# domainxz/top-k-rec

Hardware: AMD Instinct MI355X
Metric: BPR training triplets/sec (sampler + plan + step), MovieLens-10M shape (higher is better)
Workload: dtype f32

## Files before the change

### include/tkr.h

```cpp
#ifndef TKR_H
#define TKR_H
#include <stdint.h>

#ifdef __cplusplus
extern "C" {
#endif

#define TKR_VERSION 120
#define TKR_OK 0
#define TKR_E_INVAL (-1)
#define TKR_E_UNSUPPORTED (-2)
#define TKR_E_IO (-3)
#define TKR_E_PARSE (-4)
#define TKR_E_NOMEM (-5)

int tkr_version(void);
int tkr_lab_build(void);

int tkr_plan_team(int32_t batch_size);
int tkr_plan_max_blocks(int32_t batch_size);
int tkr_sample_plan(const int32_t* tr_users, int32_t n_tr, const int32_t* row_ptr, const int32_t* pos_cols,
                    const int32_t* cols_sorted, int32_t n_users, int32_t n_items, uint64_t seed,
                    uint64_t first_triplet, const int64_t* ctl, int32_t n_batches, int32_t batch_size,
                    int32_t* ucnt, int32_t* icnt, uint32_t* touch_u, uint32_t* touch_i, int32_t* out_u,
// ... 13 lines not shown
    float* b;
    float* msb;
    int32_t n_users, n_items, k;
    int32_t mode;
    float lu, li, lj, lb;
    float lr;
    float rho, eps;
    int32_t opt;
} tkr_bpr_state;

int tkr_bpr_run(const tkr_bpr_state* st, int32_t* rec, const int32_t* occ, const int32_t* hdr,
                int32_t batch_size, int32_t n_batches, float* loss_out, void* stream);

typedef struct {
    void* U;
    void* msU;
    void* tailU;
    uint32_t* rdU;
    void* V;
    void* msV;
    void* tailV;
    uint32_t* rdV;
    int32_t n_users, n_items, k;
    int32_t mode;
    float lu, li, lj, lb;
    float lr, rho, eps;
    int32_t opt;
    int32_t item_bufs;
} tkr_flow_state;
int32_t tkr_flow_row_granules(int32_t k);
int32_t tkr_flow_ctl_words(void);
#define TKR_FLOW_CTL_STATUS 1026
#define TKR_FLOW_CTL_SPINS 1027
int tkr_bpr_flow_run(const tkr_flow_state* st, const int32_t* prec, const int32_t* pocc, int32_t batch_size,
                     int32_t n_batches, uint32_t* ctl, float* loss_out, int32_t waves_per_cu, void* stream);

int32_t tkr_bpr_own_owners(int32_t n_items, int32_t k);
int32_t tkr_bpr_own_owners_shared(int32_t n_items, int32_t k, int32_t share);
int tkr_sample_plan_owned(const int32_t* tr_users, int32_t n_tr, const int32_t* row_ptr, const int32_t* pos_cols,
                          const int32_t* cols_sorted, int32_t n_users, int32_t n_items, uint64_t seed, uint64_t first_triplet,
                          int32_t n_batches, int32_t batch_size, int32_t* ucnt, int32_t* icnt, uint32_t* touch_u,
                          uint32_t* touch_i, int32_t* out_u, int32_t* out_i, int32_t* out_j, int32_t* task, int32_t* occ,
                          int32_t* occt, int32_t* prec, int32_t* pocc, int32_t n_owner, int32_t* ohdr, int32_t ohdr_stride,
                          void* stream);
int tkr_bpr_own_run(const tkr_flow_state* st, const int32_t* prec, const int32_t* pocc, const int32_t* occt, const int32_t* ohdr,
                    int32_t ohdr_stride, int32_t n_owner, int32_t batch_size, int32_t first_batch, int32_t n_batches, uint32_t* ctl, float* loss_out,
                    int32_t owner_waves, void* xch, uint32_t epoch, void* stream);
typedef struct tkr_plan_call {
    const int32_t *tr_users, *row_ptr, *pos_cols, *cols_sorted;
    int32_t *ucnt, *icnt;
    uint32_t *touch_u, *touch_i;
    int32_t *out_u, *out_i, *out_j, *task, *occ, *occt, *prec, *pocc, *ohdr;
    uint64_t seed, first_triplet;
    int32_t n_tr, n_users, n_items, n_batches, batch_size, n_owner, ohdr_stride, reserved;
} tkr_plan_call;
int tkr_bpr_own_plan_run(const tkr_plan_call* plan, const tkr_flow_state* st, int32_t first_batch, int32_t n_batches, uint32_t* ctl,
                         float* loss_out, int32_t owner_waves, void* xch, uint32_t epoch, void* ev_before, void* ev_after, void* stream);
int tkr_bpr_own_run_between(void* ev_before, void* ev_after, const tkr_flow_state* st, const int32_t* prec, const int32_t* pocc,
                            const int32_t* occt, const int32_t* ohdr, int32_t ohdr_stride, int32_t n_owner, int32_t batch_size,
                            int32_t first_batch, int32_t n_batches, uint32_t* ctl, float* loss_out, int32_t owner_waves, void* xch,
                            uint32_t epoch, void* stream);

typedef struct {
    float* U;
    float* msU;
    float* I;
// ... 246 lines not shown
```

### top-k-rec_amd/csrc/bpr_own.hip

```cpp
#include "flow_task.h"
#ifndef TKR_TAG_NAP
#define TKR_TAG_NAP 4
#endif
#ifdef TKR_PLAN_STAMP
namespace tkr { __device__ unsigned long long own_k1_prof[32]; }
#define K1_STAMP(i) do { if (blockIdx.x == 0 && threadIdx.x == 0) tkr::own_k1_prof[i] = __builtin_amdgcn_s_memrealtime(); } while (0)
#define K1_STAMP_ITEMS(i) do { if (blockIdx.x == 0 && threadIdx.x == 256) tkr::own_k1_prof[i] = __builtin_amdgcn_s_memrealtime(); } while (0)
#endif
#include "plan_parts.h"

namespace tkr {

struct PlanArgs {
    const int32_t *tr_users, *row_ptr, *pos_cols, *cols_sorted;
    int32_t *ucnt, *icnt;
    uint32_t *touch_u, *touch_i;
    int32_t *out_u, *out_i, *out_j;
    int4* task;
    int2* occ;
    int32_t* occt;
    int4 *prec, *pocc;
    int32_t* ohdr;
    uint64_t seed, first_triplet;
    uint32_t n_tr, n_items;
// ... 11 lines not shown
        }
        lds_poke(flag, ok);
    }
    __syncthreads();
    const bool ok = lds_peek(flag) != 0u;
    __syncthreads();
    return ok;
}

constexpr uint32_t kOwnInvalid = 0xffffffffu;

__host__ __device__ inline size_t plan_scratch_bytes(int B, int npad_items, int n_owner, int own_words) {
    size_t a = (size_t)npad_items * 8 + (kWideThreads / TKR_WAVE + 1) * 4;
    if (a < (size_t)(256 + 512) * 8 + 64) a = (size_t)(256 + 512) * 8 + 64;
    const size_t pb = (size_t)3 * B * 20 + (size_t)4 * n_owner * (own_words + 1) + (kWideThreads / TKR_WAVE + 1) * 4 + 16 + (size_t)3 * B * 32;
    return ((a > pb ? a : pb) + 15) & ~(size_t)15;
}

template <bool PLAN>
__device__ __forceinline__ int4 plan_ld(const int4* __restrict__ prec, const __amdgpu_buffer_rsrc_t& prec_r, size_t idx16) {
    if constexpr (PLAN) {
        const v4u x = __builtin_amdgcn_raw_buffer_load_b128(prec_r, (int)(idx16 * 16), 0, kAuxLoad);
        return make_int4((int)x.x, (int)x.y, (int)x.z, (int)x.w);
    } else {
        return prec[idx16];
    }
}
constexpr int kDotWin = 1024;

struct OwnQueue {
    uint32_t head;
    uint32_t total;
    uint32_t arrival;
    uint32_t head_batch;
};

struct QueueMap {
    const uint32_t* pre;
    const uint32_t* start;
    uint32_t slots_per_batch;
    __device__ __forceinline__ uint32_t locate(uint32_t pos, uint32_t& cur, int lane) const {
        uint32_t before;
        for (;;) {
            const uint32_t v = pre[cur + 1 + lane];
            const unsigned long long m = __ballot(v > pos);
            if (m) {
                const int f = __ffsll((long long)m) - 1;
                before = f ? (uint32_t)bcast_i((int)v, f - 1) : pre[cur];
                cur += f;
                break;
            }
            cur += TKR_WAVE;
        }
        return cur * slots_per_batch + start[cur] + (pos - before);
    }
};

template <bool PLAN>
struct UserTicketSrc {
    uint32_t ticket;
    int home, queues;
    uint32_t total;
    uint32_t B;
    const int4* __restrict__ prec;
    __amdgpu_buffer_rsrc_t prec_r;
    __device__ __forceinline__ void prefetch(NextTask& nx, int lane) {
        const u64 i64 = (u64)(uint32_t)bcast_i((int)ticket, 0) * (uint32_t)queues + (uint32_t)home;
// ... 3 lines not shown
        if (idx == 0xffffffffu) { nx.idx = idx; return; }
        nx.idx = idx + 2u * B * (idx / B);
        if (lane < 8) nx.w = plan_ld<PLAN>(prec, prec_r, (size_t)nx.idx * 8 + lane);
    }
};

template <int NP>
__device__ __forceinline__ void lds_row_read(const float* row, int lane, bool sgd, float (&own)[2 * NP], float (&ms)[2 * NP], Own& o) {
    constexpr int KP = NP * 128;
#pragma unroll
    for (int q = 0; q < NP; ++q) {
        const float2 a = *reinterpret_cast<const float2*>(row + q * 128 + 2 * lane);
        own[2 * q] = a.x; own[2 * q + 1] = a.y;
        if (!sgd) {
            const float2 m = *reinterpret_cast<const float2*>(row + KP + q * 128 + 2 * lane);
            ms[2 * q] = m.x; ms[2 * q + 1] = m.y;
        }
    }
    const float4 t = *reinterpret_cast<const float4*>(row + 2 * KP);
    const float2 t2 = *reinterpret_cast<const float2*>(row + 2 * KP + 4);
    o.b = t.x; o.msb = t.y;
    o.exp[0] = __float_as_uint(t.z); o.exp[1] = __float_as_uint(t.w);
    o.exp[2] = __float_as_uint(t2.x); o.exp[3] = __float_as_uint(t2.y);
}

struct ItemRow {
    const u64 *own_p, *own_ms, *own_tail;
    const uint32_t* own_rd;
    uint32_t ver;
    bool from_lds;
    const volatile uint32_t* tag;
    const float* row;
    int halves;
    bool rd_staged;
    uint32_t rd_val;
};

template <int NP>
__device__ __forceinline__ bool item_own_wait(const FlowTables& T, int lane, const ItemRow& r, bool sgd, float (&own)[2 * NP], float (&ms)[2 * NP],
                                              Own& o, uint32_t* ctl, uint32_t& spins) {
    if (r.from_lds) {
        uint32_t waited = 0;
        while (lds_peek(r.tag) != r.ver) {
#if TKR_TAG_NAP > 0
            __builtin_amdgcn_s_sleep(TKR_TAG_NAP);
#endif
            if (spin_fail(waited, ctl, 0)) {
                if (waited >= kSpinLimit && lane == 0 && atomicCAS(ctl + kCtlDebug, 0u, 4u) == 0u) {
                    ctl[kCtlDebug + 1] = lds_peek(r.tag); ctl[kCtlDebug + 3] = r.ver;
                }
                return false;
            }
        }
        spins += waited;
        asm volatile("" ::: "memory");
        lds_row_read<NP>(r.row, lane, sgd, own, ms, o);
        o.ok = true;
        if (r.rd_staged) {
            o.rd = r.rd_val;
            return true;
        }
    }
    return flow_own<NP>(T, lane, r.own_p, r.own_ms, r.own_tail, r.own_rd, r.ver, own, ms, o, sgd, ctl, spins, r.halves);
}

template <int NP>
struct LdsOwnStep {
    const FlowTables& T;
    int lane;
    const ItemRow& r;
    bool sgd;
    uint32_t* ctl;
    uint32_t& spins;
    __device__ __forceinline__ bool operator()(float (&own)[2 * NP], float (&ms)[2 * NP], Own& o) {
#ifdef TKR_OWN_PROF
        o.t_own0 = __builtin_amdgcn_s_memtime();
        const bool ok = item_own_wait<NP>(T, lane, r, sgd, own, ms, o, ctl, spins);
        o.t_own1 = __builtin_amdgcn_s_memtime();
        return ok;
#else
        return item_own_wait<NP>(T, lane, r, sgd, own, ms, o, ctl, spins);
#endif
    }
};
struct NoFeed {
    __device__ __forceinline__ void prefetch(NextTask& nx, int) { nx.have = true; }
};

template <int NP>
__device__ __forceinline__ void own_update(const tkr_flow_state& st, bool sgd, const float (&own)[2 * NP], const float (&ms)[2 * NP],
                                           const Own& o, const float (&g)[2 * NP], float gb, float (&pn)[2 * NP], float (&mn)[2 * NP],
                                           float& bn, float& mbn) {
    constexpr int NE = 2 * NP;
    if (sgd) {
// ... 4 lines not shown
    } else {
#pragma unroll
        for (int e = 0; e < NE; ++e) {
            mn[e] = st.rho * ms[e] + (1.f - st.rho) * g[e] * g[e];
            pn[e] = own[e] - st.lr * g[e] * __builtin_amdgcn_rsqf(mn[e] + st.eps);
        }
        mbn = st.rho * o.msb + (1.f - st.rho) * gb * gb;
        bn = o.b - st.lr * gb * __builtin_amdgcn_rsqf(mbn + st.eps);
    }
}

template <int NP>
__device__ __forceinline__ bool own_publish(int lane, bool is_item, uint32_t bmask, bool sgd, u64* tabP, u64* tabM, u64* tabT, size_t woff,
                                            size_t n_rows, int row, int rowk, uint32_t ver, int n_occ, Own& o, const uint32_t* own_rd,
                                            const float (&pn)[2 * NP], const float (&mn)[2 * NP], float bn, float mbn, uint32_t* ctl,
                                            uint32_t& spins, uint32_t readers_per_occ) {
    const uint32_t nv = ver + 1u;
    const uint32_t expect = pick_exp(o, (ver + 1u) & bmask);
    uint32_t waited = 0;
    while ((int32_t)(o.rd - expect) < 0) {
        if (spin_fail(waited, ctl)) {
            if (waited >= kSpinLimit && lane == 0 && atomicCAS(ctl + kCtlDebug, 0u, 2u) == 0u) {
                ctl[kCtlDebug + 1] = o.rd; ctl[kCtlDebug + 2] = expect; ctl[kCtlDebug + 3] = ver; ctl[kCtlDebug + 4] = (uint32_t)rowk;
            }
            return false;
        }
        o.rd = ld_u32(own_rd);
    }
    spins += waited;
#ifdef TKR_OWN_PROF
    o.t_ack = __builtin_amdgcn_s_memtime();
#endif
    store_row<NP>(tabP + woff, lane, pn, nv);
    if (!sgd) store_row<NP>(tabM + woff, lane, mn, nv);
    store_tail(tabT, n_rows, row, bmask, lane, is_item, bn, mbn, o, ver, n_occ, readers_per_occ);
    return true;
}

constexpr int own_threads(int np) { return np == 1 ? 768 : 512; }

template <int NP, bool PLAN = false>
__global__ __launch_bounds__(own_threads(NP), own_threads(NP) / 256) void bpr_own_kernel(
    tkr_flow_state st, const int4* __restrict__ prec , const int4* __restrict__ pocc,
    const int32_t* __restrict__ occt, const int32_t* __restrict__ ohdr , int ohdr_stride,
    int first_batch, int nb, int B, int n_owner, int owner_waves, uint32_t tune, uint32_t* __restrict__ ctl, float* __restrict__ loss_out,
    u64* __restrict__ xch , uint32_t epoch, PlanArgs pa) {
    constexpr int TPB = own_threads(NP);
    constexpr int NE = 2 * NP;
    constexpr int KP = NP * 128;
    constexpr int ROWF = 2 * KP + 8;
    const int lane = threadIdx.x & (TKR_WAVE - 1), wave = threadIdx.x / TKR_WAVE;
    FlowTables T;
    T.tune = 0u;
    T.kp = KP;
    T.ustride = (size_t)st.n_users * T.kp;
    T.istride = (size_t)st.n_items * T.kp;
    T.imask = st.item_bufs == 4 ? 3u : 1u;
    const int item_halves = tail_halves(T.imask);
    T.U = reinterpret_cast<u64*>(st.U); T.msU = reinterpret_cast<u64*>(st.msU); T.tailU = reinterpret_cast<u64*>(st.tailU);
    T.V = reinterpret_cast<u64*>(st.V); T.msV = reinterpret_cast<u64*>(st.msV); T.tailV = reinterpret_cast<u64*>(st.tailV);
    T.rdU = st.rdU; T.rdV = st.rdV;
    const bool sgd = st.opt == 1;
    const bool want_loss = loss_out != nullptr;

    extern __shared__ __attribute__((aligned(16))) unsigned char smem[];
    OwnQueue* q = reinterpret_cast<OwnQueue*>(smem);
    uint32_t* pre = reinterpret_cast<uint32_t*>(smem + sizeof(OwnQueue));
    uint32_t* start = pre + nb + 1 + TKR_WAVE;
    const int rows_here = (st.n_items + n_owner - 1) / n_owner;
    uint32_t* tags = start + nb;
    uint32_t* dotmark = tags + rows_here;
    float* rows = reinterpret_cast<float*>(smem + ((sizeof(OwnQueue) + (size_t)4 * (2 * nb + 1 + TKR_WAVE + rows_here + kDotWin) + 15) & ~(size_t)15));

    const uint32_t me = blockIdx.x;
    bool alive = true;
    int commit_key = -1, commit_total = 0;
#ifdef TKR_PLAN_STAMP
#define PLAN_STAMP(i) do { if ((me == 0 || me == gridDim.x - 1) && threadIdx.x == 0) reinterpret_cast<u64*>(ctl + kCtlProf)[(me ? 16 : 0) + (i)] = __builtin_amdgcn_s_memrealtime(); } while (0)
#else
#define PLAN_STAMP(i) do { } while (0)
#endif
    PLAN_STAMP(0);
    for (int b = threadIdx.x; b < TKR_WAVE; b += TPB) pre[nb + 1 + b] = 0xffffffffu;
    for (int s = threadIdx.x; s < rows_here; s += TPB) tags[s] = kOwnInvalid;
    for (int s = threadIdx.x; s < kDotWin; s += TPB) dotmark[s] = 0u;
    if constexpr (PLAN) {
        static_assert(TPB == kWideThreads, "phase B of the planner is one thread per task slot");
        unsigned char* scratch = reinterpret_cast<unsigned char*>(rows);
        volatile uint32_t* flag = &q->arrival;
        const uint32_t n_plan = (uint32_t)pa.n_plan;
        int4 ct = make_int4(-1, 0, 0, 0);
        int cprev = 0, ctotal = 0;
        if (me < n_plan) {
            const int b = (int)me, n3 = 3 * B;
            int4* task_b = pa.task + (size_t)b * n3;
            int2* occ_b = pa.occ + (size_t)b * n3;
            int32_t* occt_b = pa.occt + (size_t)b * n3;
            const bool split = pa.reg_sort_ok != 0 && pa.npad_items == 512 && B > 128;
            const PlanMirror mir = plan_mirror(scratch + plan_scratch_bytes(B, pa.npad_items, n_owner, pa.own_words), B);
            if (split)
                plan_phase_a_split<TPB>(scratch, b, pa.tr_users, pa.n_tr, pa.row_ptr, pa.pos_cols, pa.cols_sorted, pa.n_items, pa.seed,
                                        pa.first_triplet + (uint64_t)b * (uint64_t)B, B, pa.out_u + (size_t)b * B, pa.out_i + (size_t)b * B,
                                        pa.out_j + (size_t)b * B, task_b, occ_b, occt_b, pa.touch_u, pa.touch_i, mir);
            else
                plan_phase_a<TPB, 256>(scratch, b, pa.tr_users, pa.n_tr, pa.row_ptr, pa.pos_cols, pa.cols_sorted, pa.n_items, pa.seed,
                                       pa.first_triplet + (uint64_t)b * (uint64_t)B, B, pa.npad_items, pa.out_u + (size_t)b * B, pa.out_i + (size_t)b * B,
                                       pa.out_j + (size_t)b * B, task_b, occ_b, occt_b, pa.touch_u, pa.touch_i, pa.reg_sort_ok != 0);
            PLAN_STAMP(1);
            asm volatile("s_waitcnt vmcnt(0)" ::: "memory");
            __syncthreads();
            PLAN_STAMP(2);
            alive = plan_rendezvous<4>(ctl + kCtlPlanA, n_plan, true, ctl, flag);
            PLAN_STAMP(3);
            if (alive) {
                if (split)
                    plan_phase_b_wide<true, true>(scratch, b, B, task_b, occ_b, occt_b, pa.ucnt, pa.icnt, pa.touch_u, pa.touch_i, pa.pocc + (size_t)b * n3,
                                                  pa.prec + (size_t)b * n3 * 8, n_owner, pa.ohdr, ohdr_stride, pa.own_words, ct, cprev, ctotal, mir);
                else
// ... 10 lines not shown
        commit_key = (alive && me < n_plan && (int)threadIdx.x < 3 * B && ct.x != -1 && cprev == -1) ? ct.x : -1;
        commit_total = ctotal;
        PLAN_STAMP(9);
    }
    const bool ticket_wave = wave > owner_waves;
    const int tw = wave - owner_waves - 1, n_tw = TPB / TKR_WAVE - owner_waves - 1;
    const int queues = min(kQueues, max(n_tw, 1) * (int)gridDim.x);
    const int home = ticket_wave ? (int)((me * (uint32_t)n_tw + (uint32_t)tw) % (uint32_t)queues) : 0;
    uint32_t ticket = 0;
    if (ticket_wave) ticket = grab_issue(ctl, lane, home);
    for (int b = threadIdx.x; b < nb; b += TPB) {
        uint32_t h = 0u;
        if (me < (uint32_t)n_owner) {
            if constexpr (PLAN) h = (uint32_t)__hip_atomic_load(ohdr + (size_t)me * ohdr_stride + b, __ATOMIC_RELAXED, __HIP_MEMORY_SCOPE_AGENT);
            else h = (uint32_t)ohdr[(size_t)me * ohdr_stride + b];
        }
        start[b] = h & 0xffffu;
        pre[b + 1] = h >> 16;
    }
    __syncthreads();
    if (wave == 0) {
        const int per = (nb + TKR_WAVE - 1) / TKR_WAVE;
        const int b0 = min(lane * per, nb), b1 = min(b0 + per, nb);
        uint32_t mine = 0;
        for (int b = b0; b < b1; ++b) mine += pre[b + 1];
        uint32_t incl = mine;
#pragma unroll
        for (int d = 1; d < TKR_WAVE; d <<= 1) {
            const uint32_t up = (uint32_t)__shfl_up((int)incl, d);
            if (lane >= d) incl += up;
        }
        uint32_t run = incl - mine;
        for (int b = b0; b < b1; ++b) { run += pre[b + 1]; pre[b + 1] = run; }
        if (lane == TKR_WAVE - 1) { q->total = incl; q->head = 0u; q->head_batch = 0u; }
        if (lane == 0) pre[0] = 0u;
    }
    __syncthreads();

    PLAN_STAMP(10);
    uint32_t spins = 0;
#ifdef TKR_OWN_PROF
    u64 prof[16] = {0, 0, 0, 0, 0, 0, 0, 0, 0, 0, 0, 0, 0, 0, 0, 0};
    u64 tprev = __builtin_amdgcn_s_memtime();
#endif
    const QueueMap qm{pre, start, 3u * (uint32_t)B};
    const __amdgpu_buffer_rsrc_t prec_r = row_rsrc(prec, PLAN ? nb * 3 * B * 128 : 16);
    const uint32_t q_total = q->total;

    auto item_row = [&](const int4 w, ItemRow& r, int& row, int& slot) {
        const int rowk = bcast_i(w.x, 0);
        const uint32_t ver = (uint32_t)bcast_i(w.y, 0);
        const int prev = bcast_i(w.y, 1);
        row = rowk & 0x7fffffff;
        slot = row / n_owner;
        const size_t roff = (size_t)(ver & T.imask) * T.istride + (size_t)row * T.kp;
        r.own_p = T.V + roff; r.own_ms = T.msV + roff;
        r.own_tail = T.tailV + ((size_t)(ver & T.imask) * st.n_items + row) * (2 * item_halves);
        r.own_rd = T.rdV + (T.imask + 1u) * (size_t)row + ((ver + 1u) & T.imask);
        r.ver = ver;
        r.from_lds = prev >= first_batch;
        r.tag = tags + slot;
        r.row = rows + (size_t)slot * ROWF;
        r.halves = item_halves;
        r.rd_staged = false;
        r.rd_val = 0u;
    };

    constexpr uint32_t kItemReaders = 2u;
    if (wave <= owner_waves) {
        uint32_t cur = 0;
        while (alive) {
            uint32_t pos = 0;
            if (lane == 0) pos = atomicAdd(&q->head, 1u);
            pos = (uint32_t)bcast_i((int)pos, 0);
            if (pos >= q_total) break;
            const uint32_t idx = qm.locate(pos, cur, lane);
            if (lane == 0) atomicMax(&q->head_batch, cur);
            int4 w = make_int4(0, 0, 0, 0);
            if (lane < 8) w = plan_ld<PLAN>(prec, prec_r, (size_t)idx * 8 + lane);
#ifdef TKR_OWN_PROF
            asm volatile("" : "+v"(w.x) :: "memory");
            const u64 t0 = __builtin_amdgcn_s_memtime();
            prof[5] += t0 - tprev;
#endif
            ItemRow r;
            int row, slot;
            item_row(w, r, row, slot);
            const int rowk = bcast_i(w.x, 0);
            const uint32_t ver = r.ver;
            const int n_occ = bcast_i(w.z, 0), first = bcast_i(w.w, 0);
            const size_t woff = (size_t)((ver + 1u) & T.imask) * T.istride + (size_t)row * T.kp;
            float* lrow = rows + (size_t)slot * ROWF;

            float own[NE], ms[NE], g[NE];
#pragma unroll
            for (int e = 0; e < NE; ++e) { g[e] = 0.f; ms[e] = 0.f; }
            Own o = {};
            float gb = 0.f;
            o.ok = r.from_lds;
            NextTask nx;
            nx.idx = 0u; nx.w = make_int4(0, 0, 0, 0); nx.have = true;
            NoFeed feed;
            LdsOwnStep<NP> own_step{T, lane, r, sgd, ctl, spins};
            float loss_lane = 0.f;
            alive = run_task<NP, true, NoFeed, LdsOwnStep<NP>, 4>(st, T, lane, n_occ, first, w, pocc, r.own_p, r.own_ms, r.own_tail, ver, own, ms, o, g,
                                                                  gb, loss_lane, false, sgd, ctl, spins, nx, feed, own_step);
            if (!alive) break;
            if (lane == 0) dotmark[pos & (kDotWin - 1)] = pos + 1u;
#ifdef TKR_OWN_PROF
            const u64 t1 = __builtin_amdgcn_s_memtime();
#endif
            float pn[NE], mn[NE], bn, mbn;
            own_update<NP>(st, sgd, own, ms, o, g, gb, pn, mn, bn, mbn);

#pragma unroll
            for (int qq = 0; qq < NP; ++qq) {
                *reinterpret_cast<float2*>(lrow + qq * 128 + 2 * lane) = make_float2(pn[2 * qq], pn[2 * qq + 1]);
                if (!sgd) *reinterpret_cast<float2*>(lrow + KP + qq * 128 + 2 * lane) = make_float2(mn[2 * qq], mn[2 * qq + 1]);
            }
            if (lane == 0) {
                const uint32_t rb = ver & T.imask, add = kItemReaders * (uint32_t)n_occ;
                *reinterpret_cast<float4*>(lrow + 2 * KP) = make_float4(bn, mbn, __uint_as_float(o.exp[0] + (rb == 0u ? add : 0u)),
                                                                        __uint_as_float(o.exp[1] + (rb == 1u ? add : 0u)));
                *reinterpret_cast<float2*>(lrow + 2 * KP + 4) =
                    make_float2(__uint_as_float(o.exp[2] + (rb == 2u ? add : 0u)), __uint_as_float(o.exp[3] + (rb == 3u ? add : 0u)));
            }
            asm volatile("s_waitcnt lgkmcnt(0)" ::: "memory");
            if (lane == 0) lds_poke(tags + slot, ver + 1u);

            alive = own_publish<NP>(lane, true, T.imask, sgd, T.V, T.msV, T.tailV, woff, (size_t)st.n_items, row, rowk, ver, n_occ, o, r.own_rd, pn,
                                    mn, bn, mbn, ctl, spins, kItemReaders);
#ifdef TKR_OWN_PROF
            tprev = __builtin_amdgcn_s_memtime();
            prof[0] += o.t_own0 - t0; prof[1] += o.t_own1 - o.t_own0; prof[2] += t1 - o.t_own1;
            prof[3] += o.t_ack - t1; prof[4] += tprev - o.t_ack; prof[6] += 1; prof[7] += r.from_lds ? 1 : 0;
#endif
        }
    } else {
        const uint32_t total = (uint32_t)nb * (uint32_t)B;
        NextTask nx;
        nx.idx = 0u; nx.w = make_int4(0, 0, 0, 0); nx.have = false;
        while (alive) {
            if (!nx.have) {
                UserTicketSrc<PLAN> first_feed{ticket, home, queues, total, (uint32_t)B, prec, prec_r};
                first_feed.prefetch(nx, lane);
                asm volatile("" : "+v"(nx.w.x), "+v"(nx.w.y), "+v"(nx.w.z), "+v"(nx.w.w) :: "memory");
            }
            const uint32_t idx = nx.idx;
            const int4 w = nx.w;
            if (idx == 0xffffffffu) break;
            nx.have = false;
            ticket = grab_issue(ctl, lane, home);
            const int rowk = bcast_i(w.x, 0);
#ifdef TKR_OWN_PROF
            const u64 t0 = __builtin_amdgcn_s_memtime();
            prof[8] += t0 - tprev;
#endif
            if (rowk < 0) {
#ifdef TKR_OWN_PROF
                tprev = t0;
#endif
                continue;
            }
            const uint32_t ver = (uint32_t)bcast_i(w.y, 0);
            const int n_occ = bcast_i(w.z, 0);
            const int first = bcast_i(w.w, 0);
            const int batch = bcast_i(w.x, 1);
            const int row = rowk;
// ... 7 lines not shown
#pragma unroll
            for (int e = 0; e < NE; ++e) { g[e] = 0.f; ms[e] = 0.f; }
            Own o = {};
            float gb = 0.f, loss_lane = 0.f;
            UserTicketSrc<PLAN> feed{ticket, home, queues, total, (uint32_t)B, prec, prec_r};
            GlobalOwn<NP> own_step{T, lane, T.U + roff, T.msU + roff, own_tail, own_rd, ver, sgd, ctl, spins, 2};
            alive = run_task<NP, false, UserTicketSrc<PLAN>, GlobalOwn<NP>, 4>(st, T, lane, n_occ, first, w, pocc, T.U + roff, T.msU + roff, own_tail, ver,
                                                                         own, ms, o, g, gb, loss_lane, want_loss, sgd, ctl, spins, nx, feed, own_step);
            if (!alive) break;
#ifdef TKR_OWN_PROF
            const u64 t1 = __builtin_amdgcn_s_memtime();
#endif
            if (want_loss) {
                const float tot = wave_sum(loss_lane);
                if (lane == 0) {
                    const uint32_t slot = idx - (uint32_t)(batch - first_batch) * 3u * (uint32_t)B;
                    __hip_atomic_store(xch + ((size_t)batch * B + slot) * 2, ((u64)epoch << 32) | (u64)__float_as_uint(tot), __ATOMIC_RELAXED,
                                       __HIP_MEMORY_SCOPE_AGENT);
                }
            }
            float pn[NE], mn[NE], bn, mbn;
            own_update<NP>(st, sgd, own, ms, o, g, gb, pn, mn, bn, mbn);
            asm volatile("" : "+v"(nx.w.x), "+v"(nx.w.y), "+v"(nx.w.z), "+v"(nx.w.w));
            alive = own_publish<NP>(lane, false, 1u, sgd, T.U, T.msU, T.tailU, woff, (size_t)st.n_users, row, rowk, ver, n_occ, o, own_rd, pn, mn,
                                    bn, mbn, ctl, spins, 2u);
#ifdef TKR_OWN_PROF
            tprev = __builtin_amdgcn_s_memtime();
            prof[9] += t1 - t0; prof[11] += o.t_ack - t1; prof[12] += tprev - o.t_ack; prof[13] += 1;
#endif
        }
    }

    if (lane == 0 && spins) atomicAdd(ctl + kCtlSpins, spins);
#ifdef TKR_OWN_PROF
    if (lane == 0)
        for (int qq = 0; qq < 16; ++qq) atomicAdd(reinterpret_cast<u64*>(ctl + kCtlProf) + qq, prof[qq]);
#endif
    asm volatile("s_waitcnt vmcnt(0)" ::: "memory");
    __syncthreads();
    PLAN_STAMP(11);
    if constexpr (PLAN) {
        if (commit_key != -1) plan_commit_first_touch(make_int4(commit_key, 0, 0, 0), -1, commit_total, pa.ucnt, pa.icnt, pa.touch_u, pa.touch_i);
    }
    const bool fold_loss = want_loss && (tune & 8u) != 0u;
    if (threadIdx.x == 0) {
        const bool last = __hip_atomic_fetch_add(ctl + kCtlLeave, 1u, __ATOMIC_RELAXED, __HIP_MEMORY_SCOPE_AGENT) == gridDim.x - 1u;
        if (last) {
            for (int qq = 0; qq < kQueues; ++qq) ctl[qq * kQueueStride] = 0u;
            ctl[kCtlArrive] = 0u;
            ctl[kCtlLeave] = 0u;
            if constexpr (PLAN) { ctl[kCtlPlanA] = 0u; ctl[kCtlPlanB] = 0u; ctl[kCtlPlanC] = 0u; }
        }
        q->arrival = last ? 1u : 0u;
    }
    if (!fold_loss) return;
    __syncthreads();
    if (q->arrival == 0u) return;
    for (int b = wave; b < nb; b += TPB / TKR_WAVE) {
        const int batch = first_batch + b;
        float part[4];
#pragma unroll
        for (int w = 0; w < 4; ++w) {
            float acc = 0.f;
            for (int t = w * TKR_WAVE + lane; t < B; t += 256) {
                const u64 g = __hip_atomic_load(xch + ((size_t)batch * B + t) * 2, __ATOMIC_RELAXED, __HIP_MEMORY_SCOPE_AGENT);
                if ((uint32_t)(g >> 32) == epoch) acc += __uint_as_float((uint32_t)g);
            }
            part[w] = wave_sum(acc);
        }
// ... 52 lines not shown
    if (st->opt == 0 && (!st->msU || !st->msV)) return TKR_EINVAL;
    if (st->n_users <= 0 || st->n_items <= 0 || st->k <= 0) return TKR_EINVAL;
    if (st->k > 256) return TKR_EUNSUPPORTED;
    if (st->item_bufs != 0 && st->item_bufs != 2 && st->item_bufs != 4) return TKR_EINVAL;
    if (!xch || epoch == 0u) return TKR_EINVAL;
    if (!prec || !pocc || !occt || !ohdr || !ctl || batch_size <= 0 || n_batches < 0 || first_batch < 0 || n_owner <= 0) return TKR_EINVAL;
    if (ohdr_stride < first_batch + n_batches || n_batches > 512) return TKR_EINVAL;
    if (n_batches == 0) return TKR_OK;
    if ((uint64_t)(first_batch + n_batches) * 3u * (uint64_t)batch_size >= 0xffffffffull / 8) return TKR_EUNSUPPORTED;
    const int np = (st->k + 127) / 128;
    int dev = 0;
    TKR_CHECK(hipGetDevice(&dev));
    static int cached_cus[64];
    static bool attr_set[64][3];
    int cus;
    if (dev >= 0 && dev < 64 && cached_cus[dev] > 0) cus = cached_cus[dev];
    else {
        TKR_CHECK(hipDeviceGetAttribute(&cus, hipDeviceAttributeMultiprocessorCount, dev));
        if (dev >= 0 && dev < 64) cached_cus[dev] = cus;
    }
    if (n_owner > cus) return TKR_EUNSUPPORTED;
    size_t lds = tkr::own_lds_bytes(np, n_batches, st->n_items, n_owner);
    if (pa) lds = tkr::own_lds_bytes_planned(np, n_batches, st->n_items, n_owner, batch_size, pa->npad_items, pa->own_words);
    if (lds > 160 * 1024) return TKR_EUNSUPPORTED;
    const uint32_t tune = ((uint32_t)owner_waves >> 8) & 0xffu;
    owner_waves &= 0xff;
    if ((tune & (1u | 128u)) || (np == 1 && (tune & (32u | 64u)))) return TKR_EUNSUPPORTED;
    if (pa && np != 1) return TKR_EINVAL;
    const int tpb = tkr::own_threads(np);
    const int waves = tpb / TKR_WAVE;
    int ow = owner_waves > 0 ? owner_waves : (waves == 12 ? 9 : 6);
    if (ow < 1) ow = 1;
    if (ow > waves - 2) ow = waves - 2;
    const bool fold = loss_out && n_batches <= 64 && !(tune & 2u);
    const uint32_t ktune = (tune & ~8u) | (fold ? 8u : 0u);
    const void* fn = pa ? (const void*)tkr::bpr_own_kernel<1, true>
                   : np == 1 ? (const void*)tkr::bpr_own_kernel<1, false> : (const void*)tkr::bpr_own_kernel<2, false>;
    const int form = pa ? 2 : np - 1;
    if (lds > 64 * 1024 && !(dev >= 0 && dev < 64 && attr_set[dev][form])) {
        TKR_CHECK(hipFuncSetAttribute(fn, hipFuncAttributeMaxDynamicSharedMemorySize, 160 * 1024));
        if (dev >= 0 && dev < 64) attr_set[dev][form] = true;
    }
    static signed char fits[64][3];
    if (dev >= 0 && dev < 64 && fits[dev][form] == 0) {
        int per_cu = 0;
        TKR_CHECK(hipOccupancyMaxActiveBlocksPerMultiprocessor(&per_cu, fn, tpb, 160 * 1024));
        fits[dev][form] = per_cu >= 1 ? 1 : -1;
    }
    if (dev >= 0 && dev < 64 && fits[dev][form] < 0) return TKR_EUNSUPPORTED;
    hipStream_t s = (hipStream_t)stream;
    const int4* r4 = reinterpret_cast<const int4*>(prec) + (size_t)first_batch * 3 * batch_size * 8;
    const int4* o4 = reinterpret_cast<const int4*>(pocc);
    ohdr += first_batch;
    const tkr::PlanArgs no_plan = {};
#define TKR_OWN_LAUNCH(NPV, PL)                                                                                                           \
    hipLaunchKernelGGL((tkr::bpr_own_kernel<NPV, PL>), dim3(n_owner), dim3(tkr::own_threads(NPV)), lds, s, *st, r4, o4, occt, ohdr, ohdr_stride,   \
                       first_batch, n_batches, batch_size, n_owner, ow, ktune, ctl, loss_out, static_cast<tkr::u64*>(xch), epoch, PL ? *pa : no_plan)
    if (pa) TKR_OWN_LAUNCH(1, true);
    else if (np == 1) TKR_OWN_LAUNCH(1, false);
    else TKR_OWN_LAUNCH(2, false);
#undef TKR_OWN_LAUNCH
    TKR_LAUNCH_CHECK();
    if (loss_out && !fold) {
        hipLaunchKernelGGL(tkr::own_loss_kernel, dim3(n_batches), dim3(256), 0, s, static_cast<const tkr::u64*>(xch), first_batch, batch_size, epoch,
                           loss_out);
        TKR_LAUNCH_CHECK();
    }
    return TKR_OK;
}

extern "C" int tkr_bpr_own_run(const tkr_flow_state* st, const int32_t* prec, const int32_t* pocc, const int32_t* occt, const int32_t* ohdr,
                               int32_t ohdr_stride, int32_t n_owner, int32_t batch_size, int32_t first_batch, int32_t n_batches,
                               uint32_t* ctl, float* loss_out, int32_t owner_waves, void* xch, uint32_t epoch, void* stream) {
    return own_launch(st, prec, pocc, occt, ohdr, ohdr_stride, n_owner, batch_size, first_batch, n_batches, ctl, loss_out, owner_waves, xch, epoch,
                      nullptr, stream);
}

extern "C" int tkr_bpr_own_run_between(void* ev_before, void* ev_after, const tkr_flow_state* st, const int32_t* prec, const int32_t* pocc,
                                       const int32_t* occt, const int32_t* ohdr, int32_t ohdr_stride, int32_t n_owner, int32_t batch_size,
                                       int32_t first_batch, int32_t n_batches, uint32_t* ctl, float* loss_out, int32_t owner_waves, void* xch,
                                       uint32_t epoch, void* stream) {
    if (ev_before) TKR_CHECK(hipEventRecord((hipEvent_t)ev_before, (hipStream_t)stream));
    const int rc = tkr_bpr_own_run(st, prec, pocc, occt, ohdr, ohdr_stride, n_owner, batch_size, first_batch, n_batches, ctl, loss_out, owner_waves,
                                   xch, epoch, stream);
    if (ev_after) TKR_CHECK(hipEventRecord((hipEvent_t)ev_after, (hipStream_t)stream));
    return rc;
}

extern "C" int tkr_bpr_own_plan_run(const tkr_plan_call* plan, const tkr_flow_state* st, int32_t first_batch, int32_t n_batches, uint32_t* ctl,
                                    float* loss_out, int32_t owner_waves, void* xch, uint32_t epoch, void* ev_before, void* ev_after,
// ... 49 lines not shown
```

### top-k-rec_amd/csrc/flow_task.h

```cpp
#pragma once
#include <stdlib.h>

#include "tkr_common.h"
#include "../../include/tkr.h"

namespace tkr {

typedef unsigned long long u64;

constexpr int kQueues = 32;
constexpr int kQueueStride = 32;
constexpr int kCtlArrive = kQueues * kQueueStride;
constexpr int kCtlLeave = kCtlArrive + 1;
constexpr int kCtlStatus = kCtlArrive + 2;
constexpr int kCtlSpins = kCtlArrive + 3;
constexpr int kCtlPlanA = kCtlArrive + 4;
constexpr int kCtlPlanB = kCtlArrive + 5;
constexpr int kCtlPlanC = kCtlArrive + 6;
constexpr int kCtlDebug = kCtlArrive + 8;
constexpr int kCtlProf = kCtlArrive + 32;
constexpr uint32_t kSpinLimit = 1u << 20;

typedef uint32_t v4u __attribute__((ext_vector_type(4)));
typedef uint32_t v2u __attribute__((ext_vector_type(2)));

constexpr int kAuxLoad = 16;
constexpr int kAuxStore = 16;
__device__ __forceinline__ __amdgpu_buffer_rsrc_t row_rsrc(const void* p, int bytes) {
    return __builtin_amdgcn_make_buffer_rsrc(const_cast<void*>(p), 0, bytes, 0x00020000);
}
__device__ __forceinline__ uint32_t ld_u32(const uint32_t* p) {
    return __hip_atomic_load(p, __ATOMIC_RELAXED, __HIP_MEMORY_SCOPE_AGENT);
}

template <int NP>
__device__ __forceinline__ void issue_row(const u64* __restrict__ row, int lane, v4u (&x)[NP]) {
    const __amdgpu_buffer_rsrc_t r = row_rsrc(row, NP * 1024);
#pragma unroll
    for (int q = 0; q < NP; ++q) x[q] = __builtin_amdgcn_raw_buffer_load_b128(r, q * 1024 + lane * 16, 0, kAuxLoad);
}
template <int NP>
__device__ __forceinline__ bool row_tagged(const v4u (&x)[NP], uint32_t tag) {
    bool ok = true;
#pragma unroll
    for (int q = 0; q < NP; ++q) ok &= (x[q].y == tag) & (x[q].w == tag);
    return ok;
}
template <int NP>
__device__ __forceinline__ void row_values(const v4u (&x)[NP], float (&v)[2 * NP]) {
#pragma unroll
    for (int q = 0; q < NP; ++q) {
        v[2 * q] = __uint_as_float(x[q].x);
// ... 429 lines not shown
    } else {
        dotv = reduce_multi<G>(part, lane);
    }
    const float bd = ITEM ? o.b - pk.bias_me : pk.bias_me;
    const float x_me = (ITEM && pk.role_me) ? -(bd + dotv) : (bd + dotv);
    const float s_me = fast_sigmoid_neg(x_me);
    if constexpr (!ITEM) {
        if (want_loss) {
            if (myq < pk.n && (lane & ((1 << SH) - 1)) == 0) loss_lane += softplus_neg(x_me);
            float own_part = 0.f;
#pragma unroll
            for (int e = 0; e < NE; ++e) own_part += l2 ? 0.5f * own[e] * own[e] * st.lu : fabsf(own[e]) * st.lu;
            loss_lane += pk.loss_part + (float)pk.n * own_part;
        }
    }
#pragma unroll
    for (int q = 0; q < G; ++q) {
        if (q < pk.n) {
            const float s = bcast_f(s_me, q << SH);
            float sg = -s;
            if constexpr (ITEM) {
                if ((pk.roles >> q) & 1u) sg = s;
                gb += sg;
            }
#pragma unroll
            for (int e = 0; e < NE; ++e) g[e] = fmaf(sg, pk.pa[q][e], g[e]);
        }
    }
#pragma unroll
    for (int e = 0; e < NE; ++e) g[e] = fmaf(pk.lam_sum, l2 ? own[e] : sgn(own[e]), g[e]);
    if constexpr (ITEM) gb = fmaf((float)pk.n * st.lb, l2 ? o.b : sgn(o.b), gb);
}

template <int NP>
struct GlobalOwn {
    const FlowTables& T;
    int lane;
    const u64 *own_p, *own_ms, *own_tail;
    const uint32_t* own_rd;
    uint32_t ver;
    bool sgd;
    uint32_t* ctl;
    uint32_t& spins;
    int own_halves;
    __device__ __forceinline__ bool operator()(float (&own)[2 * NP], float (&ms)[2 * NP], Own& o) {
        return flow_own<NP>(T, lane, own_p, own_ms, own_tail, own_rd, ver, own, ms, o, sgd, ctl, spins, own_halves);
    }
};

template <int NP, bool ITEM, class Src, class OwnStep, int KBIG = 8>
__device__ __forceinline__ bool run_task(const tkr_flow_state& st, const FlowTables& T, int lane, int n_occ, int first, const int4 w,
                                         const int4* __restrict__ pocc, const u64* own_p, const u64* own_ms, const u64* own_tail,
                                         uint32_t ver, float (&own)[2 * NP], float (&ms)[2 * NP], Own& o,
                                         float (&g)[2 * NP], float& gb, float& loss_lane, bool want_loss, bool sgd, uint32_t* ctl,
                                         uint32_t& spins, NextTask& nx, Src& feed, OwnStep& own_step) {
#define TKR_FETCH(GG, nn, dd, PK)                                                                                                  \
    flow_fetch<NP, GG, ITEM>(st, T, lane, nn, dd, own_p, own_ms, own_tail, ver, own, ms, o, want_loss, sgd, ctl, spins, nx, feed, PK)
#define TKR_ONE(GG, nn, dd)                                                                                    \
    {                                                                                                          \
        Packed<NP, GG> pk;                                                                                     \
        if (!TKR_FETCH(GG, nn, dd, pk)) return false;                                                          \
        if (!own_step(own, ms, o)) return false;                                                               \
        flow_apply<NP, GG, ITEM>(st, T, lane, pk, own, o, g, gb, loss_lane, want_loss);                          \
        return true;                                                                                           \
    }
    if (n_occ <= 4) {
        const int src = (lane + 2) & 7;
        const int4 d = make_int4(__shfl(w.x, src), __shfl(w.y, src), __shfl(w.z, src), __shfl(w.w, src));
        switch (n_occ) {
            case 1: TKR_ONE(1, 1, d)
            case 2: TKR_ONE(2, 2, d)
            case 3: TKR_ONE(3, 3, d)
            default: TKR_ONE(4, 4, d)
        }
    }
    constexpr int kBig = KBIG;
    static_assert(kBig == 4 || kBig == 8, "round width");
    if (n_occ <= 2 * kBig) {
        const int n0 = min(kBig, n_occ), n1 = n_occ - n0;
        int4 d0 = make_int4(0, 0, 0, 0), d1 = make_int4(0, 0, 0, 0);
        if (lane < n0) d0 = pocc[first + lane];
        if (lane < n1) d1 = pocc[first + kBig + lane];
        Packed<NP, kBig> p0, p1;
        if (!TKR_FETCH(kBig, n0, d0, p0)) return false;
        if (n1 > 0 && !TKR_FETCH(kBig, n1, d1, p1)) return false;
        if (!own_step(own, ms, o)) return false;
        flow_apply<NP, kBig, ITEM>(st, T, lane, p0, own, o, g, gb, loss_lane, want_loss);
        if (n1 > 0) flow_apply<NP, kBig, ITEM>(st, T, lane, p1, own, o, g, gb, loss_lane, want_loss);
        return true;
    }
    for (int done = 0; done < n_occ; done += kBig) {
        const int n = min(kBig, n_occ - done);
        int4 d = make_int4(0, 0, 0, 0);
        if (lane < n) d = pocc[first + done + lane];
        Packed<NP, kBig> pk;
        if (!TKR_FETCH(kBig, n, d, pk)) return false;
        if (done == 0 && !own_step(own, ms, o)) return false;
        flow_apply<NP, kBig, ITEM>(st, T, lane, pk, own, o, g, gb, loss_lane, want_loss);
    }
    return true;
#undef TKR_ONE
#undef TKR_FETCH
}

}
```

### top-k-rec_amd/tkr_hip.py

```python
from __future__ import annotations

import ctypes as C
import warnings
import os

import torch

_HERE = os.path.dirname(os.path.abspath(__file__))
LIB_PATH = os.environ.get('TKR_HIP_LIB') or os.path.join(_HERE, 'libtkr_hip.so')

_lib = None
VERSION = 120


class TkrError(RuntimeError):
    pass


class StepGaveUp(TkrError):
    """a bounded spin of a persistent step kernel ran out: the tables of the run are invalid, the engine has stepped down to the
    next kernel (K2o -> K2f -> K2) and works again once valid tables are put back (BPR.train does)"""


class BprState(C.Structure):
# ... 216 lines not shown


def plan_rollback(plan, B, first_batch, n_batches, cnt):
    _call('tkr_plan_rollback', plan.task, _p(plan.task), C.c_int32(B), C.c_int32(first_batch), C.c_int32(n_batches),
                                   _p(cnt.ucnt), _p(cnt.icnt))


def _at(t, offset):
    if t is None:
        return C.c_void_p(0)
    assert t.is_cuda and t.is_contiguous() and 0 <= offset <= t.numel()
    return C.c_void_p(t.data_ptr() + offset * t.element_size())


def bpr_run(state, plan, B, n_batches, loss_out=None, first=0):
    rs = plan_max_blocks(B) * plan_team(B) * 16
    _call('tkr_bpr_run', plan.rec, C.byref(state), _at(plan.rec, first * rs), _at(plan.occ, first * 6 * B), _at(plan.hdr, first * 4),
                             C.c_int32(B), C.c_int32(n_batches), _at(loss_out, first))


FLOW_MAX_K = 256


def flow_row_granules(k):
    return int(lib().tkr_flow_row_granules(C.c_int32(k)))


def flow_ctl_words():
    return int(lib().tkr_flow_ctl_words())


FLOW_CTL_ARRIVE, FLOW_CTL_STATUS, FLOW_CTL_SPINS = 1024, 1026, 1027
FLOW_CTL_DEBUG, FLOW_CTL_PROF = 1032, 1056


def bpr_flow_run(state, plan, B, n_batches, ctl, loss_out=None, first=0, waves_per_cu=0):
    _call('tkr_bpr_flow_run', plan.prec, C.byref(state), _at(plan.prec, first * 3 * B * 32), _p(plan.pocc), C.c_int32(B),
          C.c_int32(n_batches), _p(ctl), _p(loss_out), C.c_int32(waves_per_cu))


def flow_stepper(state, B, ctl, waves_per_cu=0):
    fn = lib().tkr_bpr_flow_run
    fn.argtypes = [C.c_void_p, C.c_void_p, C.c_void_p, C.c_int32, C.c_int32, C.c_void_p, C.c_void_p, C.c_int32, C.c_void_p]
    device, st = ctl.device, C.addressof(state)
    ctl_ptr, rec_bytes = ctl.data_ptr(), 3 * B * 32 * 4

    def step(plan, first, n_batches, loss_out):
        if torch.cuda.current_device() != device.index:
            return bpr_flow_run(state, plan, B, n_batches, ctl, loss_out, first, waves_per_cu)
        rc = fn(st, plan.prec.data_ptr() + first * rec_bytes, plan.pocc.data_ptr(), B, n_batches, ctl_ptr,
                None if loss_out is None else loss_out.data_ptr(), waves_per_cu, torch.cuda.current_stream(device).cuda_stream)
        if rc:
            _check(rc, 'tkr_bpr_flow_run')
    step.state = state
    return step


def bpr_own_owners(n_items, k, device=None, share=1):
    if device is not None and torch.cuda.current_device() != device.index:
        with torch.cuda.device(device):
            return int(lib().tkr_bpr_own_owners_shared(C.c_int32(n_items), C.c_int32(k), C.c_int32(share)))
    return int(lib().tkr_bpr_own_owners_shared(C.c_int32(n_items), C.c_int32(k), C.c_int32(share)))


def bpr_own_run(state, plan, B, n_batches, ctl, loss_out=None, first=0, owner_waves=0):
    plan.epoch += 1
# ... 1331 lines not shown
```

Measured before the change: 43.31 million.

## Stash extra fetch rounds in LDS so more tasks prefetch before owner wait

```diff
diff --git a/include/tkr.h b/include/tkr.h
--- a/include/tkr.h
+++ b/include/tkr.h
@@ -69,6 +69,8 @@
 int32_t tkr_flow_ctl_words(void);
 #define TKR_FLOW_CTL_STATUS 1026
 #define TKR_FLOW_CTL_SPINS 1027
+#define TKR_FLOW_CTL_STASH_USED 1048
+#define TKR_FLOW_CTL_STASH_FELL 1049
 int tkr_bpr_flow_run(const tkr_flow_state* st, const int32_t* prec, const int32_t* pocc, int32_t batch_size,
                      int32_t n_batches, uint32_t* ctl, float* loss_out, int32_t waves_per_cu, void* stream);
 
diff --git a/top-k-rec_amd/csrc/bpr_own.hip b/top-k-rec_amd/csrc/bpr_own.hip
--- a/top-k-rec_amd/csrc/bpr_own.hip
+++ b/top-k-rec_amd/csrc/bpr_own.hip
@@ -67,7 +67,7 @@
     uint32_t head;
     uint32_t total;
     uint32_t arrival;
-    uint32_t head_batch;
+    uint32_t stash_busy;
 };
 
 struct QueueMap {
@@ -137,8 +137,6 @@
     const volatile uint32_t* tag;
     const float* row;
     int halves;
-    bool rd_staged;
-    uint32_t rd_val;
 };
 
 template <int NP>
@@ -161,10 +159,6 @@
         asm volatile("" ::: "memory");
         lds_row_read<NP>(r.row, lane, sgd, own, ms, o);
         o.ok = true;
-        if (r.rd_staged) {
-            o.rd = r.rd_val;
-            return true;
-        }
     }
     return flow_own<NP>(T, lane, r.own_p, r.own_ms, r.own_tail, r.own_rd, r.ver, own, ms, o, sgd, ctl, spins, r.halves);
 }
@@ -235,8 +229,8 @@
     o.t_ack = __builtin_amdgcn_s_memtime();
 #endif
     store_row<NP>(tabP + woff, lane, pn, nv);
+    store_tail(tabT, n_rows, row, bmask, lane, is_item, bn, mbn, o, ver, n_occ, readers_per_occ);
     if (!sgd) store_row<NP>(tabM + woff, lane, mn, nv);
-    store_tail(tabT, n_rows, row, bmask, lane, is_item, bn, mbn, o, ver, n_occ, readers_per_occ);
     return true;
 }
 
@@ -247,7 +241,8 @@
     tkr_flow_state st, const int4* __restrict__ prec , const int4* __restrict__ pocc,
     const int32_t* __restrict__ occt, const int32_t* __restrict__ ohdr , int ohdr_stride,
     int first_batch, int nb, int B, int n_owner, int owner_waves, uint32_t tune, uint32_t* __restrict__ ctl, float* __restrict__ loss_out,
-    u64* __restrict__ xch , uint32_t epoch, PlanArgs pa) {
+    u64* __restrict__ xch , uint32_t epoch,
+    int stash_off , int stash_slots, PlanArgs pa) {
     constexpr int TPB = own_threads(NP);
     constexpr int NE = 2 * NP;
     constexpr int KP = NP * 128;
@@ -272,7 +267,6 @@
     uint32_t* start = pre + nb + 1 + TKR_WAVE;
     const int rows_here = (st.n_items + n_owner - 1) / n_owner;
     uint32_t* tags = start + nb;
-    uint32_t* dotmark = tags + rows_here;
     float* rows = reinterpret_cast<float*>(smem + ((sizeof(OwnQueue) + (size_t)4 * (2 * nb + 1 + TKR_WAVE + rows_here + kDotWin) + 15) & ~(size_t)15));
 
     const uint32_t me = blockIdx.x;
@@ -286,7 +280,6 @@
     PLAN_STAMP(0);
     for (int b = threadIdx.x; b < TKR_WAVE; b += TPB) pre[nb + 1 + b] = 0xffffffffu;
     for (int s = threadIdx.x; s < rows_here; s += TPB) tags[s] = kOwnInvalid;
-    for (int s = threadIdx.x; s < kDotWin; s += TPB) dotmark[s] = 0u;
     if constexpr (PLAN) {
         static_assert(TPB == kWideThreads, "phase B of the planner is one thread per task slot");
         unsigned char* scratch = reinterpret_cast<unsigned char*>(rows);
@@ -363,15 +356,16 @@
         }
         uint32_t run = incl - mine;
         for (int b = b0; b < b1; ++b) { run += pre[b + 1]; pre[b + 1] = run; }
-        if (lane == TKR_WAVE - 1) { q->total = incl; q->head = 0u; q->head_batch = 0u; }
+        if (lane == TKR_WAVE - 1) { q->total = incl; q->head = 0u; q->stash_busy = 0u; }
         if (lane == 0) pre[0] = 0u;
     }
     __syncthreads();
 
     PLAN_STAMP(10);
     uint32_t spins = 0;
-#ifdef TKR_OWN_PROF
-    u64 prof[16] = {0, 0, 0, 0, 0, 0, 0, 0, 0, 0, 0, 0, 0, 0, 0, 0};
+    LdsStash<NP> stash{reinterpret_cast<float*>(smem + stash_off), &q->stash_busy, stash_slots, wave, lane, 0u, 0u, nullptr, 0u};
+#ifdef TKR_OWN_PROF
+    u64 prof[24] = {0, 0, 0, 0, 0, 0, 0, 0, 0, 0, 0, 0, 0, 0, 0, 0, 0, 0, 0, 0, 0, 0, 0, 0};
     u64 tprev = __builtin_amdgcn_s_memtime();
 #endif
     const QueueMap qm{pre, start, 3u * (uint32_t)B};
@@ -393,8 +387,6 @@
         r.tag = tags + slot;
         r.row = rows + (size_t)slot * ROWF;
         r.halves = item_halves;
-        r.rd_staged = false;
-        r.rd_val = 0u;
     };
 
     constexpr uint32_t kItemReaders = 2u;
@@ -406,7 +398,6 @@
             pos = (uint32_t)bcast_i((int)pos, 0);
             if (pos >= q_total) break;
             const uint32_t idx = qm.locate(pos, cur, lane);
-            if (lane == 0) atomicMax(&q->head_batch, cur);
             int4 w = make_int4(0, 0, 0, 0);
             if (lane < 8) w = plan_ld<PLAN>(prec, prec_r, (size_t)idx * 8 + lane);
 #ifdef TKR_OWN_PROF
@@ -434,10 +425,9 @@
             NoFeed feed;
             LdsOwnStep<NP> own_step{T, lane, r, sgd, ctl, spins};
             float loss_lane = 0.f;
-            alive = run_task<NP, true, NoFeed, LdsOwnStep<NP>, 4>(st, T, lane, n_occ, first, w, pocc, r.own_p, r.own_ms, r.own_tail, ver, own, ms, o, g,
-                                                                  gb, loss_lane, false, sgd, ctl, spins, nx, feed, own_step);
+            alive = run_task<NP, true, NoFeed, LdsOwnStep<NP>, 4, LdsStash<NP>>(st, T, lane, n_occ, first, w, pocc, r.own_p, r.own_ms, r.own_tail, ver, own,
+                                                                                ms, o, g, gb, loss_lane, false, sgd, ctl, spins, nx, feed, own_step, stash);
             if (!alive) break;
-            if (lane == 0) dotmark[pos & (kDotWin - 1)] = pos + 1u;
 #ifdef TKR_OWN_PROF
             const u64 t1 = __builtin_amdgcn_s_memtime();
 #endif
@@ -465,6 +455,8 @@
             tprev = __builtin_amdgcn_s_memtime();
             prof[0] += o.t_own0 - t0; prof[1] += o.t_own1 - o.t_own0; prof[2] += t1 - o.t_own1;
             prof[3] += o.t_ack - t1; prof[4] += tprev - o.t_ack; prof[6] += 1; prof[7] += r.from_lds ? 1 : 0;
+            const int cls = n_occ <= 4 ? 0 : n_occ <= 8 ? 1 : n_occ <= 16 ? 2 : 3;
+            prof[16 + 2 * cls] += t1 - o.t_own1; prof[17 + 2 * cls] += 1;
 #endif
         }
     } else {
@@ -538,9 +530,11 @@
     }
 
     if (lane == 0 && spins) atomicAdd(ctl + kCtlSpins, spins);
+    if (lane == 0 && stash.used) atomicAdd(ctl + kCtlStashUsed, stash.used);
+    if (lane == 0 && stash.fell) atomicAdd(ctl + kCtlStashFell, stash.fell);
 #ifdef TKR_OWN_PROF
     if (lane == 0)
-        for (int qq = 0; qq < 16; ++qq) atomicAdd(reinterpret_cast<u64*>(ctl + kCtlProf) + qq, prof[qq]);
+        for (int qq = 0; qq < 24; ++qq) atomicAdd(reinterpret_cast<u64*>(ctl + kCtlProf) + qq, prof[qq]);
 #endif
     asm volatile("s_waitcnt vmcnt(0)" ::: "memory");
     __syncthreads();
@@ -659,6 +653,11 @@
     int ow = owner_waves > 0 ? owner_waves : (waves == 12 ? 9 : 6);
     if (ow < 1) ow = 1;
     if (ow > waves - 2) ow = waves - 2;
+    const int stash_off = (int)lds;
+    int stash_slots = (int)((160 * 1024 - lds) / tkr::stash_slot_bytes(np));
+    if (stash_slots > ow + 1) stash_slots = ow + 1;
+    if (tune & 4u) stash_slots = 0;
+    lds += (size_t)stash_slots * tkr::stash_slot_bytes(np);
     const bool fold = loss_out && n_batches <= 64 && !(tune & 2u);
     const uint32_t ktune = (tune & ~8u) | (fold ? 8u : 0u);
     const void* fn = pa ? (const void*)tkr::bpr_own_kernel<1, true>
@@ -682,7 +681,8 @@
     const tkr::PlanArgs no_plan = {};
 #define TKR_OWN_LAUNCH(NPV, PL)                                                                                                           \
     hipLaunchKernelGGL((tkr::bpr_own_kernel<NPV, PL>), dim3(n_owner), dim3(tkr::own_threads(NPV)), lds, s, *st, r4, o4, occt, ohdr, ohdr_stride,   \
-                       first_batch, n_batches, batch_size, n_owner, ow, ktune, ctl, loss_out, static_cast<tkr::u64*>(xch), epoch, PL ? *pa : no_plan)
+                       first_batch, n_batches, batch_size, n_owner, ow, ktune, ctl, loss_out, static_cast<tkr::u64*>(xch), epoch, stash_off, stash_slots,    \
+                       PL ? *pa : no_plan)
     if (pa) TKR_OWN_LAUNCH(1, true);
     else if (np == 1) TKR_OWN_LAUNCH(1, false);
     else TKR_OWN_LAUNCH(2, false);
diff --git a/top-k-rec_amd/csrc/flow_task.h b/top-k-rec_amd/csrc/flow_task.h
--- a/top-k-rec_amd/csrc/flow_task.h
+++ b/top-k-rec_amd/csrc/flow_task.h
@@ -18,6 +18,8 @@
 constexpr int kCtlPlanB = kCtlArrive + 5;
 constexpr int kCtlPlanC = kCtlArrive + 6;
 constexpr int kCtlDebug = kCtlArrive + 8;
+constexpr int kCtlStashUsed = kCtlArrive + 24;
+constexpr int kCtlStashFell = kCtlArrive + 25;
 constexpr int kCtlProf = kCtlArrive + 32;
 constexpr uint32_t kSpinLimit = 1u << 20;
 
@@ -513,6 +515,76 @@
     if constexpr (ITEM) gb = fmaf((float)pk.n * st.lb, l2 ? o.b : sgn(o.b), gb);
 }
 
+struct NoStash {
+    static constexpr bool enabled = false;
+    __device__ __forceinline__ bool claim() { return false; }
+    __device__ __forceinline__ void release() {}
+    template <class PK> __device__ __forceinline__ void put(int, const PK&) {}
+    template <class PK> __device__ __forceinline__ void get(int, PK&) {}
+};
+
+typedef __attribute__((address_space(3))) uint32_t lds_u32_t;
+typedef __attribute__((address_space(3))) float lds_f32_t;
+
+constexpr int stash_round_floats(int np) { return (8 * np + 6) * 64 + 4; }
+constexpr int kStashRounds = 2;
+constexpr size_t stash_slot_bytes(int np) { return (size_t)kStashRounds * stash_round_floats(np) * 4; }
+
+template <int NP>
+struct LdsStash {
+    static constexpr bool enabled = true;
+    float* slots;
+    uint32_t* busy;
+    int n_slots, wave, lane;
+    uint32_t used, fell;
+    float* mine;
+    uint32_t bit;
+    __device__ __forceinline__ bool claim() {
+        uint32_t got = 0u;
+        if (n_slots > 0) {
+            const int s = wave % n_slots;
+            bit = 1u << s;
+            mine = slots + (size_t)s * (kStashRounds * stash_round_floats(NP));
+            if (lane == 0) got = (__hip_atomic_fetch_or((lds_u32_t*)busy, bit, __ATOMIC_RELAXED, __HIP_MEMORY_SCOPE_WORKGROUP) & bit) ? 0u : 1u;
+            got = (uint32_t)bcast_i((int)got, 0);
+        }
+        if (got) ++used; else ++fell;
+        return got != 0u;
+    }
+    __device__ __forceinline__ void release() {
+        asm volatile("s_waitcnt lgkmcnt(0)" ::: "memory");
+        if (lane == 0) __hip_atomic_fetch_and((lds_u32_t*)busy, ~bit, __ATOMIC_RELAXED, __HIP_MEMORY_SCOPE_WORKGROUP);
+    }
+    __device__ __forceinline__ void put(int r, const Packed<NP, 4>& pk) {
+        lds_f32_t* p = (lds_f32_t*)(mine + r * stash_round_floats(NP)) + lane;
+        int w = 0;
+#pragma unroll
+        for (int q = 0; q < 4; ++q) {
+#pragma unroll
+            for (int e = 0; e < 2 * NP; ++e) p[64 * w++] = pk.pa[q][e];
+            p[64 * w++] = pk.c[q];
+        }
+        p[64 * w++] = pk.bias_me;
+        p[64 * w++] = pk.role_me ? 1.f : 0.f;
+        if (lane == 0) { p[64 * w] = __uint_as_float(pk.roles); p[64 * w + 1] = pk.lam_sum; p[64 * w + 2] = __int_as_float(pk.n); }
+    }
+    __device__ __forceinline__ void get(int r, Packed<NP, 4>& pk) {
+        const lds_f32_t* p = (const lds_f32_t*)(mine + r * stash_round_floats(NP)) + lane;
+        int w = 0;
+#pragma unroll
+        for (int q = 0; q < 4; ++q) {
+#pragma unroll
+            for (int e = 0; e < 2 * NP; ++e) pk.pa[q][e] = p[64 * w++];
+            pk.c[q] = p[64 * w++];
+        }
+        pk.bias_me = p[64 * w++];
+        pk.role_me = p[64 * w++] != 0.f;
+        const lds_f32_t* u = p + 64 * w - lane;
+        pk.roles = (uint32_t)bcast_i(__float_as_int(u[0]), 0); pk.lam_sum = bcast_f(u[1], 0); pk.n = bcast_i(__float_as_int(u[2]), 0);
+        pk.loss_part = 0.f;
+    }
+};
+
 template <int NP>
 struct GlobalOwn {
     const FlowTables& T;
@@ -529,12 +601,12 @@
     }
 };
 
-template <int NP, bool ITEM, class Src, class OwnStep, int KBIG = 8>
+template <int NP, bool ITEM, class Src, class OwnStep, int KBIG, class Stash>
 __device__ __forceinline__ bool run_task(const tkr_flow_state& st, const FlowTables& T, int lane, int n_occ, int first, const int4 w,
                                          const int4* __restrict__ pocc, const u64* own_p, const u64* own_ms, const u64* own_tail,
                                          uint32_t ver, float (&own)[2 * NP], float (&ms)[2 * NP], Own& o,
                                          float (&g)[2 * NP], float& gb, float& loss_lane, bool want_loss, bool sgd, uint32_t* ctl,
-                                         uint32_t& spins, NextTask& nx, Src& feed, OwnStep& own_step) {
+                                         uint32_t& spins, NextTask& nx, Src& feed, OwnStep& own_step, Stash& stash) {
 #define TKR_FETCH(GG, nn, dd, PK)                                                                                                  \
     flow_fetch<NP, GG, ITEM>(st, T, lane, nn, dd, own_p, own_ms, own_tail, ver, own, ms, o, want_loss, sgd, ctl, spins, nx, feed, PK)
 #define TKR_ONE(GG, nn, dd)                                                                                    \
@@ -557,8 +629,24 @@
     }
     constexpr int kBig = KBIG;
     static_assert(kBig == 4 || kBig == 8, "round width");
-    if (n_occ <= 2 * kBig) {
-        const int n0 = min(kBig, n_occ), n1 = n_occ - n0;
+    bool ahead = n_occ <= 2 * kBig;
+    if constexpr (Stash::enabled) {
+        static_assert(kBig == 4, "the stash holds Packed<NP, 4>");
+        if (!ahead && n_occ <= (2 + kStashRounds) * kBig) ahead = stash.claim();
+    }
+    if (ahead) {
+        int n_st = 0;
+        if constexpr (Stash::enabled) {
+            for (int done = 2 * kBig; done < n_occ; done += kBig, ++n_st) {
+                const int n = min(kBig, n_occ - done);
+                int4 d = make_int4(0, 0, 0, 0);
+                if (lane < n) d = pocc[first + done + lane];
+                Packed<NP, kBig> pk;
+                if (!TKR_FETCH(kBig, n, d, pk)) return false;
+                stash.put(n_st, pk);
+            }
+        }
+        const int n0 = min(kBig, n_occ), n1 = min(kBig, n_occ - n0);
         int4 d0 = make_int4(0, 0, 0, 0), d1 = make_int4(0, 0, 0, 0);
         if (lane < n0) d0 = pocc[first + lane];
         if (lane < n1) d1 = pocc[first + kBig + lane];
@@ -568,6 +656,16 @@
         if (!own_step(own, ms, o)) return false;
         flow_apply<NP, kBig, ITEM>(st, T, lane, p0, own, o, g, gb, loss_lane, want_loss);
         if (n1 > 0) flow_apply<NP, kBig, ITEM>(st, T, lane, p1, own, o, g, gb, loss_lane, want_loss);
+        if constexpr (Stash::enabled) {
+            if (n_st > 0) {
+                for (int r = 0; r < n_st; ++r) {
+                    Packed<NP, kBig> pk;
+                    stash.get(r, pk);
+                    flow_apply<NP, kBig, ITEM>(st, T, lane, pk, own, o, g, gb, loss_lane, want_loss);
+                }
+                stash.release();
+            }
+        }
         return true;
     }
     for (int done = 0; done < n_occ; done += kBig) {
@@ -583,5 +681,15 @@
 #undef TKR_ONE
 #undef TKR_FETCH
 }
-
-}
+template <int NP, bool ITEM, class Src, class OwnStep, int KBIG = 8>
+__device__ __forceinline__ bool run_task(const tkr_flow_state& st, const FlowTables& T, int lane, int n_occ, int first, const int4 w,
+                                         const int4* __restrict__ pocc, const u64* own_p, const u64* own_ms, const u64* own_tail,
+                                         uint32_t ver, float (&own)[2 * NP], float (&ms)[2 * NP], Own& o,
+                                         float (&g)[2 * NP], float& gb, float& loss_lane, bool want_loss, bool sgd, uint32_t* ctl,
+                                         uint32_t& spins, NextTask& nx, Src& feed, OwnStep& own_step) {
+    NoStash none;
+    return run_task<NP, ITEM, Src, OwnStep, KBIG, NoStash>(st, T, lane, n_occ, first, w, pocc, own_p, own_ms, own_tail, ver, own, ms, o, g, gb, loss_lane,
+                                                           want_loss, sgd, ctl, spins, nx, feed, own_step, none);
+}
+
+}
diff --git a/top-k-rec_amd/tkr_hip.py b/top-k-rec_amd/tkr_hip.py
--- a/top-k-rec_amd/tkr_hip.py
+++ b/top-k-rec_amd/tkr_hip.py
@@ -272,6 +272,8 @@
 
 FLOW_CTL_ARRIVE, FLOW_CTL_STATUS, FLOW_CTL_SPINS = 1024, 1026, 1027
 FLOW_CTL_DEBUG, FLOW_CTL_PROF = 1032, 1056
+FLOW_CTL_STASH_USED, FLOW_CTL_STASH_FELL = 1048, 1049
+OWN_TUNE_NO_STASH = 0x400
 
 
 def bpr_flow_run(state, plan, B, n_batches, ctl, loss_out=None, first=0, waves_per_cu=0):
```

Result: slower. 42.78 million (-1.2%).
